# EternityJune25/ComoRAG

Measured on NVIDIA H100. Metric: queries/sec, higher is better.
Workload: dtype bf16

## Files before the change

comorag_b200/csrc/attention_tc.cu:

```cuda
#include <cstdlib>

#include "common.cuh"
#include "encoder.cuh"
#include "ptx.cuh"

namespace crag {

constexpr int kAttBM = 128;
constexpr int kAttBN = 64;
constexpr int kAttDH = 64;
constexpr int kAttThreads = 288;
constexpr int kAttTileBytes = 128 * 64 * 2;
constexpr int kAttKVBytes = kAttBN * 64 * 2;
constexpr size_t kAttSmemBytes = 1024 + kAttTileBytes + 4 * kAttKVBytes + 256;

__device__ __forceinline__ float att_exp2(float x) {
  float y;
  asm("ex2.approx.ftz.f32 %0, %1;" : "=f"(y) : "f"(x));
  return y;
}

__device__ __forceinline__ uint32_t att_pack_bf16x2(float a, float b) {
  __nv_bfloat162 v = __floats2bfloat162_rn(a, b);
  return *reinterpret_cast<uint32_t*>(&v);
}

__global__ void __launch_bounds__(kAttThreads, 1)
attention_tc_kernel(const __grid_constant__ CUtensorMap tm_q, const __grid_constant__ CUtensorMap tm_kv,
                    const int32_t* __restrict__ cu_seqlens, int H, float scale_log2e, __nv_bfloat16* __restrict__ ctx) {
  const int seq = blockIdx.z, head = blockIdx.y;
  const int start = __ldg(cu_seqlens + seq);
  const int L = __ldg(cu_seqlens + seq + 1) - start;
  const int q0 = blockIdx.x * kAttBM;
  if (q0 >= L) return;
  const int n_blk = (L + kAttBN - 1) / kAttBN;

  extern __shared__ uint8_t smem_raw[];
  uint8_t* smem = reinterpret_cast<uint8_t*>((reinterpret_cast<uintptr_t>(smem_raw) + 1023) & ~uintptr_t(1023));
  uint8_t* sQ = smem;
  uint8_t* sK = sQ + kAttTileBytes;
  uint8_t* sV = sK + 2 * kAttKVBytes;
  uint64_t* bar_q = reinterpret_cast<uint64_t*>(sV + 2 * kAttKVBytes);
  uint64_t* bar_k_full = bar_q + 1;
  uint64_t* bar_v_full = bar_k_full + 2;
  uint64_t* bar_kv_empty = bar_v_full + 2;

  const int warp = threadIdx.x >> 5, lane = threadIdx.x & 31;
  if (threadIdx.x == 0) {
    mbar_init(bar_q, 1);
    for (int s = 0; s < 2; ++s) {
      mbar_init(&bar_k_full[s], 1);
      mbar_init(&bar_v_full[s], 1);
      mbar_init(&bar_kv_empty[s], 8);
    }
    fence_mbar_init();
  }
  __syncthreads();

  if (warp == 8) {
    if (lane == 0) {
      tma_prefetch_desc(&tm_q);
      tma_prefetch_desc(&tm_kv);
      mbar_arrive_expect_tx(bar_q, kAttTileBytes);
      tma_load_2d(&tm_q, bar_q, sQ, head * kAttDH, start + q0);
      for (int j = 0; j < n_blk; ++j) {
        const int st = j & 1;
        const uint32_t ph = (j >> 1) & 1;
        mbar_wait(&bar_kv_empty[st], ph ^ 1);
        mbar_arrive_expect_tx(&bar_k_full[st], kAttKVBytes);
        tma_load_2d(&tm_kv, &bar_k_full[st], sK + st * kAttKVBytes, H + head * kAttDH, start + j * kAttBN);
        mbar_arrive_expect_tx(&bar_v_full[st], kAttKVBytes);
        tma_load_2d(&tm_kv, &bar_v_full[st], sV + st * kAttKVBytes, 2 * H + head * kAttDH, start + j * kAttBN);
      }
    }
    return;
  }

  const int wg = warp >> 2;
  const uint32_t q_addr = smem_u32(sQ) + wg * 64 * 128;
  float o[32];
#pragma unroll
  for (int i = 0; i < 32; ++i) o[i] = 0.f;
  float m_run[2] = {-INFINITY, -INFINITY}, l_run[2] = {0.f, 0.f};
  mbar_wait(bar_q, 0);
  for (int j = 0; j < n_blk; ++j) {
    const int st = j & 1;
    const uint32_t ph = (j >> 1) & 1;
    mbar_wait(&bar_k_full[st], ph);
    float s[32];
    const uint32_t k_addr = smem_u32(sK + st * kAttKVBytes);
    wgmma_fence();
#pragma unroll
    for (int ks = 0; ks < kAttDH / 16; ++ks)
      wgmma_m64n64k16_ss(s, wgmma_desc_sw128(q_addr + ks * 32), wgmma_desc_sw128(k_addr + ks * 32), ks > 0 ? 1u : 0u);
    wgmma_commit();
    wgmma_wait<0>();
    wgmma_fence_regs(s);

    const int kbase = j * kAttBN + 2 * (lane & 3);
    if (j * kAttBN + kAttBN > L) {
#pragma unroll
      for (int c = 0; c < 8; ++c)
#pragma unroll
        for (int e = 0; e < 2; ++e)
          if (kbase + 8 * c + e >= L) s[4 * c + e] = s[4 * c + 2 + e] = -INFINITY;
    }
    float alpha[2];
#pragma unroll
    for (int h = 0; h < 2; ++h) {
      float mx = -INFINITY;
#pragma unroll
      for (int c = 0; c < 8; ++c) mx = fmaxf(mx, fmaxf(s[4 * c + 2 * h], s[4 * c + 2 * h + 1]));
      mx = fmaxf(mx, __shfl_xor_sync(0xffffffffu, mx, 1));
      mx = fmaxf(mx, __shfl_xor_sync(0xffffffffu, mx, 2));
      const float m_new = fmaxf(m_run[h], mx * scale_log2e);
      alpha[h] = att_exp2(m_run[h] - m_new);
      m_run[h] = m_new;
    }
    uint32_t pa[4][4];
    float rs[2] = {0.f, 0.f};
#pragma unroll
    for (int c = 0; c < 8; ++c) {
#pragma unroll
      for (int h = 0; h < 2; ++h) {
        const float p0 = att_exp2(fmaf(s[4 * c + 2 * h], scale_log2e, -m_run[h]));
        const float p1 = att_exp2(fmaf(s[4 * c + 2 * h + 1], scale_log2e, -m_run[h]));
        rs[h] += p0 + p1;
        pa[c >> 1][(c & 1) * 2 + h] = att_pack_bf16x2(p0, p1);
      }
    }
#pragma unroll
    for (int h = 0; h < 2; ++h) l_run[h] = l_run[h] * alpha[h] + rs[h];
#pragma unroll
    for (int c = 0; c < 8; ++c) {
      o[4 * c + 0] *= alpha[0];
      o[4 * c + 1] *= alpha[0];
      o[4 * c + 2] *= alpha[1];
      o[4 * c + 3] *= alpha[1];
    }
    mbar_wait(&bar_v_full[st], ph);
    const uint32_t v_addr = smem_u32(sV + st * kAttKVBytes);
    wgmma_fence();
#pragma unroll
    for (int kk = 0; kk < kAttBN / 16; ++kk)
      wgmma_m64n64k16_rs_bmn(o, pa[kk], wgmma_desc_sw128(v_addr + kk * 16 * 128), 1u);
    wgmma_commit();
    wgmma_wait<0>();
    wgmma_fence_regs(o);
    __syncwarp();
    if (lane == 0) mbar_arrive(&bar_kv_empty[st]);
  }

#pragma unroll
  for (int h = 0; h < 2; ++h) {
    float l = l_run[h];
    l += __shfl_xor_sync(0xffffffffu, l, 1);
    l += __shfl_xor_sync(0xffffffffu, l, 2);
    const float inv = 1.f / l;
    const int row = q0 + wg * 64 + (warp & 3) * 16 + (lane >> 2) + 8 * h;
    if (row < L) {
      __nv_bfloat16* dst = ctx + int64_t(start + row) * H + head * kAttDH + 2 * (lane & 3);
#pragma unroll
      for (int c = 0; c < 8; ++c)
        *reinterpret_cast<uint32_t*>(dst + 8 * c) = att_pack_bf16x2(o[4 * c + 2 * h] * inv, o[4 * c + 2 * h + 1] * inv);
    }
  }
}

int launch_attention_tc(const void* qkv, const int32_t* cu_seqlens, int n_seqs, int total_tokens, int max_len, int H,
                        int heads, void* ctx, cudaStream_t stream) {
  if (n_seqs <= 0 || max_len <= 0 || total_tokens <= 0) return CRAG_OK;
  if (H / heads != kAttDH) return fail(CRAG_ERR_UNSUPPORTED, "attention_tc: head dim must be 64");
  CUtensorMap tm_q, tm_kv;
  int rc = make_tmap_bf16_2d(&tm_q, qkv, uint64_t(total_tokens), uint64_t(3) * H, uint64_t(3) * H * 2, kAttBM);
  if (rc != CRAG_OK) return rc;
  rc = make_tmap_bf16_2d(&tm_kv, qkv, uint64_t(total_tokens), uint64_t(3) * H, uint64_t(3) * H * 2, kAttBN);
  if (rc != CRAG_OK) return rc;
  const dim3 grid((max_len + kAttBM - 1) / kAttBM, heads, n_seqs);
  const float scale_log2e = 1.4426950408889634f / sqrtf(float(kAttDH));
  rc = allow_dynamic_smem<attention_tc_kernel>(kAttSmemBytes);
  if (rc != CRAG_OK) return rc;
  attention_tc_kernel<<<grid, kAttThreads, kAttSmemBytes, stream>>>(tm_q, tm_kv, cu_seqlens, H, scale_log2e,
                                                                    static_cast<__nv_bfloat16*>(ctx));
  CRAG_CUDA_OK(cudaGetLastError());
  return CRAG_OK;
}

}
```

Before: 4607.

## Overlap QK^T and PV wgmma across iterations with deeper TMA pipeline

Restructures the attention main loop so the S=QK^T wgmma for block j+1 is issued together with the PV wgmma for block j, letting softmax of the next block overlap tensor-core work. The dedicated producer warp is removed; thread 0 of the consumer warps now issues TMA loads inline. The K/V ring grows from 2 to 5 stages, with separate empty barriers for K and V. The goal is to hide wgmma latency and the softmax critical path, at the cost of more shared memory, more live registers, and TMA issue stalls on the consumer thread.

```diff
diff --git a/comorag_b200/csrc/attention_tc.cu b/comorag_b200/csrc/attention_tc.cu
--- a/comorag_b200/csrc/attention_tc.cu
+++ b/comorag_b200/csrc/attention_tc.cu
@@ -9,10 +9,11 @@
 constexpr int kAttBM = 128;
 constexpr int kAttBN = 64;
 constexpr int kAttDH = 64;
-constexpr int kAttThreads = 288;
+constexpr int kAttThreads = 256;
+constexpr int kAttStages = 5;
 constexpr int kAttTileBytes = 128 * 64 * 2;
 constexpr int kAttKVBytes = kAttBN * 64 * 2;
-constexpr size_t kAttSmemBytes = 1024 + kAttTileBytes + 4 * kAttKVBytes + 256;
+constexpr size_t kAttSmemBytes = 1024 + kAttTileBytes + 2 * kAttStages * kAttKVBytes + 256;
 
 __device__ __forceinline__ float att_exp2(float x) {
   float y;
@@ -23,6 +24,78 @@
 __device__ __forceinline__ uint32_t att_pack_bf16x2(float a, float b) {
   __nv_bfloat162 v = __floats2bfloat162_rn(a, b);
   return *reinterpret_cast<uint32_t*>(&v);
+}
+
+__device__ __forceinline__ void att_softmax(float (&s)[32], int j, int L, int lane, float scale_log2e, float (&m_run)[2],
+                                            float (&l_run)[2], float (&alpha)[2], float (&p)[32]) {
+  const int kbase = j * kAttBN + 2 * (lane & 3);
+  if (j * kAttBN + kAttBN > L) {
+#pragma unroll
+    for (int c = 0; c < 8; ++c)
+#pragma unroll
+      for (int e = 0; e < 2; ++e)
+        if (kbase + 8 * c + e >= L) s[4 * c + e] = s[4 * c + 2 + e] = -INFINITY;
+  }
+#pragma unroll
+  for (int h = 0; h < 2; ++h) {
+    float mx = -INFINITY;
+#pragma unroll
+    for (int c = 0; c < 8; ++c) mx = fmaxf(mx, fmaxf(s[4 * c + 2 * h], s[4 * c + 2 * h + 1]));
+    mx = fmaxf(mx, __shfl_xor_sync(0xffffffffu, mx, 1));
+    mx = fmaxf(mx, __shfl_xor_sync(0xffffffffu, mx, 2));
+    const float m_new = fmaxf(m_run[h], mx * scale_log2e);
+    alpha[h] = att_exp2(m_run[h] - m_new);
+    m_run[h] = m_new;
+  }
+  float rs[2] = {0.f, 0.f};
+#pragma unroll
+  for (int c = 0; c < 8; ++c) {
+#pragma unroll
+    for (int h = 0; h < 2; ++h) {
+      const float p0 = att_exp2(fmaf(s[4 * c + 2 * h], scale_log2e, -m_run[h]));
+      const float p1 = att_exp2(fmaf(s[4 * c + 2 * h + 1], scale_log2e, -m_run[h]));
+      rs[h] += p0 + p1;
+      p[4 * c + 2 * h] = p0;
+      p[4 * c + 2 * h + 1] = p1;
+    }
+  }
+#pragma unroll
+  for (int h = 0; h < 2; ++h) l_run[h] = l_run[h] * alpha[h] + rs[h];
+}
+
+__device__ __forceinline__ void att_pack(const float (&p)[32], uint32_t (&pa)[4][4]) {
+#pragma unroll
+  for (int c = 0; c < 8; ++c)
+#pragma unroll
+    for (int h = 0; h < 2; ++h) pa[c >> 1][(c & 1) * 2 + h] = att_pack_bf16x2(p[4 * c + 2 * h], p[4 * c + 2 * h + 1]);
+}
+
+__device__ __forceinline__ void att_rescale(float (&o)[32], const float (&alpha)[2]) {
+#pragma unroll
+  for (int c = 0; c < 8; ++c) {
+    o[4 * c + 0] *= alpha[0];
+    o[4 * c + 1] *= alpha[0];
+    o[4 * c + 2] *= alpha[1];
+    o[4 * c + 3] *= alpha[1];
+  }
+}
+
+__device__ __forceinline__ void att_issue_s(float (&s)[32], uint32_t q_addr, uint32_t k_addr) {
+#pragma unroll
+  for (int ks = 0; ks < kAttDH / 16; ++ks)
+    wgmma_m64n64k16_ss(s, wgmma_desc_sw128(q_addr + ks * 32), wgmma_desc_sw128(k_addr + ks * 32), ks > 0 ? 1u : 0u);
+  wgmma_commit();
+}
+
+__device__ __forceinline__ void att_issue_pv(float (&o)[32], const uint32_t (&pa)[4][4], uint32_t v_addr) {
+#pragma unroll
+  for (int kk = 0; kk < kAttBN / 16; ++kk) wgmma_m64n64k16_rs_bmn(o, pa[kk], wgmma_desc_sw128(v_addr + kk * 16 * 128), 1u);
+  wgmma_commit();
+}
+
+__device__ __forceinline__ void att_release(uint64_t* bar, int lane) {
+  __syncwarp();
+  if (lane == 0) mbar_arrive(bar);
 }
 
 __global__ void __launch_bounds__(kAttThreads, 1)
@@ -39,42 +112,49 @@
   uint8_t* smem = reinterpret_cast<uint8_t*>((reinterpret_cast<uintptr_t>(smem_raw) + 1023) & ~uintptr_t(1023));
   uint8_t* sQ = smem;
   uint8_t* sK = sQ + kAttTileBytes;
-  uint8_t* sV = sK + 2 * kAttKVBytes;
-  uint64_t* bar_q = reinterpret_cast<uint64_t*>(sV + 2 * kAttKVBytes);
+  uint8_t* sV = sK + kAttStages * kAttKVBytes;
+  uint64_t* bar_q = reinterpret_cast<uint64_t*>(sV + kAttStages * kAttKVBytes);
   uint64_t* bar_k_full = bar_q + 1;
-  uint64_t* bar_v_full = bar_k_full + 2;
-  uint64_t* bar_kv_empty = bar_v_full + 2;
+  uint64_t* bar_v_full = bar_k_full + kAttStages;
+  uint64_t* bar_k_empty = bar_v_full + kAttStages;
+  uint64_t* bar_v_empty = bar_k_empty + kAttStages;
 
   const int warp = threadIdx.x >> 5, lane = threadIdx.x & 31;
-  if (threadIdx.x == 0) {
+  const bool producer = threadIdx.x == 0;
+  const auto load_k = [&](int b) {
+    const int st = b % kAttStages;
+    if (b >= kAttStages) mbar_wait(&bar_k_empty[st], ((b / kAttStages) - 1) & 1);
+    mbar_arrive_expect_tx(&bar_k_full[st], kAttKVBytes);
+    tma_load_2d(&tm_kv, &bar_k_full[st], sK + st * kAttKVBytes, H + head * kAttDH, start + b * kAttBN);
+  };
+  const auto load_v = [&](int b) {
+    const int st = b % kAttStages;
+    if (b >= kAttStages) mbar_wait(&bar_v_empty[st], ((b / kAttStages) - 1) & 1);
+    mbar_arrive_expect_tx(&bar_v_full[st], kAttKVBytes);
+    tma_load_2d(&tm_kv, &bar_v_full[st], sV + st * kAttKVBytes, 2 * H + head * kAttDH, start + b * kAttBN);
+  };
+  if (producer) {
     mbar_init(bar_q, 1);
-    for (int s = 0; s < 2; ++s) {
+    for (int s = 0; s < kAttStages; ++s) {
       mbar_init(&bar_k_full[s], 1);
       mbar_init(&bar_v_full[s], 1);
-      mbar_init(&bar_kv_empty[s], 8);
+      mbar_init(&bar_k_empty[s], 8);
+      mbar_init(&bar_v_empty[s], 8);
     }
     fence_mbar_init();
   }
   __syncthreads();
-
-  if (warp == 8) {
-    if (lane == 0) {
-      tma_prefetch_desc(&tm_q);
-      tma_prefetch_desc(&tm_kv);
-      mbar_arrive_expect_tx(bar_q, kAttTileBytes);
-      tma_load_2d(&tm_q, bar_q, sQ, head * kAttDH, start + q0);
-      for (int j = 0; j < n_blk; ++j) {
-        const int st = j & 1;
-        const uint32_t ph = (j >> 1) & 1;
-        mbar_wait(&bar_kv_empty[st], ph ^ 1);
-        mbar_arrive_expect_tx(&bar_k_full[st], kAttKVBytes);
-        tma_load_2d(&tm_kv, &bar_k_full[st], sK + st * kAttKVBytes, H + head * kAttDH, start + j * kAttBN);
-        mbar_arrive_expect_tx(&bar_v_full[st], kAttKVBytes);
-        tma_load_2d(&tm_kv, &bar_v_full[st], sV + st * kAttKVBytes, 2 * H + head * kAttDH, start + j * kAttBN);
-      }
-    }
-    return;
-  }
+  if (producer) {
+    tma_prefetch_desc(&tm_q);
+    tma_prefetch_desc(&tm_kv);
+    mbar_arrive_expect_tx(bar_q, kAttTileBytes);
+    tma_load_2d(&tm_q, bar_q, sQ, head * kAttDH, start + q0);
+    for (int b = 0; b < kAttStages && b < n_blk; ++b) {
+      load_k(b);
+      load_v(b);
+    }
+  }
+  __syncwarp();
 
   const int wg = warp >> 2;
   const uint32_t q_addr = smem_u32(sQ) + wg * 64 * 128;
@@ -82,73 +162,53 @@
 #pragma unroll
   for (int i = 0; i < 32; ++i) o[i] = 0.f;
   float m_run[2] = {-INFINITY, -INFINITY}, l_run[2] = {0.f, 0.f};
+  float s[32], alpha[2];
+  uint32_t pa[4][4];
   mbar_wait(bar_q, 0);
-  for (int j = 0; j < n_blk; ++j) {
-    const int st = j & 1;
-    const uint32_t ph = (j >> 1) & 1;
-    mbar_wait(&bar_k_full[st], ph);
-    float s[32];
-    const uint32_t k_addr = smem_u32(sK + st * kAttKVBytes);
-    wgmma_fence();
-#pragma unroll
-    for (int ks = 0; ks < kAttDH / 16; ++ks)
-      wgmma_m64n64k16_ss(s, wgmma_desc_sw128(q_addr + ks * 32), wgmma_desc_sw128(k_addr + ks * 32), ks > 0 ? 1u : 0u);
-    wgmma_commit();
-    wgmma_wait<0>();
-    wgmma_fence_regs(s);
-
-    const int kbase = j * kAttBN + 2 * (lane & 3);
-    if (j * kAttBN + kAttBN > L) {
-#pragma unroll
-      for (int c = 0; c < 8; ++c)
-#pragma unroll
-        for (int e = 0; e < 2; ++e)
-          if (kbase + 8 * c + e >= L) s[4 * c + e] = s[4 * c + 2 + e] = -INFINITY;
-    }
-    float alpha[2];
-#pragma unroll
-    for (int h = 0; h < 2; ++h) {
-      float mx = -INFINITY;
-#pragma unroll
-      for (int c = 0; c < 8; ++c) mx = fmaxf(mx, fmaxf(s[4 * c + 2 * h], s[4 * c + 2 * h + 1]));
-      mx = fmaxf(mx, __shfl_xor_sync(0xffffffffu, mx, 1));
-      mx = fmaxf(mx, __shfl_xor_sync(0xffffffffu, mx, 2));
-      const float m_new = fmaxf(m_run[h], mx * scale_log2e);
-      alpha[h] = att_exp2(m_run[h] - m_new);
-      m_run[h] = m_new;
-    }
-    uint32_t pa[4][4];
-    float rs[2] = {0.f, 0.f};
-#pragma unroll
-    for (int c = 0; c < 8; ++c) {
-#pragma unroll
-      for (int h = 0; h < 2; ++h) {
-        const float p0 = att_exp2(fmaf(s[4 * c + 2 * h], scale_log2e, -m_run[h]));
-        const float p1 = att_exp2(fmaf(s[4 * c + 2 * h + 1], scale_log2e, -m_run[h]));
-        rs[h] += p0 + p1;
-        pa[c >> 1][(c & 1) * 2 + h] = att_pack_bf16x2(p0, p1);
-      }
-    }
-#pragma unroll
-    for (int h = 0; h < 2; ++h) l_run[h] = l_run[h] * alpha[h] + rs[h];
-#pragma unroll
-    for (int c = 0; c < 8; ++c) {
-      o[4 * c + 0] *= alpha[0];
-      o[4 * c + 1] *= alpha[0];
-      o[4 * c + 2] *= alpha[1];
-      o[4 * c + 3] *= alpha[1];
-    }
-    mbar_wait(&bar_v_full[st], ph);
-    const uint32_t v_addr = smem_u32(sV + st * kAttKVBytes);
-    wgmma_fence();
-#pragma unroll
-    for (int kk = 0; kk < kAttBN / 16; ++kk)
-      wgmma_m64n64k16_rs_bmn(o, pa[kk], wgmma_desc_sw128(v_addr + kk * 16 * 128), 1u);
-    wgmma_commit();
+
+  float p[32];
+  mbar_wait(&bar_k_full[0], 0);
+  wgmma_fence();
+  att_issue_s(s, q_addr, smem_u32(sK));
+  wgmma_wait<0>();
+  wgmma_fence_regs(s);
+  att_release(&bar_k_empty[0], lane);
+  att_softmax(s, 0, L, lane, scale_log2e, m_run, l_run, alpha, p);
+
+  for (int j = 0; j + 1 < n_blk; ++j) {
+    const int sk = (j + 1) % kAttStages, sv = j % kAttStages;
     wgmma_wait<0>();
     wgmma_fence_regs(o);
+    if (j > 0) att_release(&bar_v_empty[(j - 1) % kAttStages], lane);
+    att_pack(p, pa);
+    att_rescale(o, alpha);
+    if (producer) {
+      if (j >= 1 && j - 1 + kAttStages < n_blk) load_k(j - 1 + kAttStages);
+      if (j >= 2 && j - 2 + kAttStages < n_blk) load_v(j - 2 + kAttStages);
+    }
     __syncwarp();
-    if (lane == 0) mbar_arrive(&bar_kv_empty[st]);
+    mbar_wait(&bar_k_full[sk], ((j + 1) / kAttStages) & 1);
+    mbar_wait(&bar_v_full[sv], (j / kAttStages) & 1);
+    wgmma_fence();
+    att_issue_s(s, q_addr, smem_u32(sK + sk * kAttKVBytes));
+    att_issue_pv(o, pa, smem_u32(sV + sv * kAttKVBytes));
+    wgmma_wait<1>();
+    wgmma_fence_regs(s);
+    att_release(&bar_k_empty[sk], lane);
+    att_softmax(s, j + 1, L, lane, scale_log2e, m_run, l_run, alpha, p);
+  }
+
+  {
+    const int sv = (n_blk - 1) % kAttStages;
+    wgmma_wait<0>();
+    wgmma_fence_regs(o);
+    att_pack(p, pa);
+    att_rescale(o, alpha);
+    mbar_wait(&bar_v_full[sv], ((n_blk - 1) / kAttStages) & 1);
+    wgmma_fence();
+    att_issue_pv(o, pa, smem_u32(sV + sv * kAttKVBytes));
+    wgmma_wait<0>();
+    wgmma_fence_regs(o);
   }
 
 #pragma unroll
```

After: 4604, median of 6. About the same (-0.1%).
